# joshspeagle/dynesty

Measured on AMD Instinct MI355X. Metric: proposals/sec + ellipsoid-rebuilds/sec, 25-D corr-Normal nlive=2000 (multi/rwalk), higher is better.
Workload: dtype f64; 1 GPU; C2 x 64 independent runs per GPU (C5 shard); per step and run: 1 MultiEllipsoid rebuild + enlarge 1.25 + 4 queue fills of K=512 walkers x 45 rwalk steps (= one bound-update interval at the queue size that passes the ln Z gate); live sets uniform inside the likelihood contour; ndim=25, nlive=2000, walks=45, queue_size=512, runs_per_gpu=64, tap_point=A (kernel boundary), rebuild_in_step=True, rng=PCG64 + ziggurat, stream-identical to numpy.random.Generator (parity mode)

## Files before the change

### dynesty_amd/csrc/rebuild.hip

```cpp
#include <math.h>
#include <stdlib.h>

#include "ctx.h"
#include <type_traits>
#include <vector>
#include "eig_wave.h"
#include "rebuild_plan.h"

using namespace dh;
using namespace dh_plan;
using dh_eig::jacobi_wave;
using dh_eig::sort_eigs_wave;
using dh_eig::wave_sync;

namespace {

constexpr double kRoundDelta = 1e-3;
constexpr double kMaxCond = 1e12;
constexpr double kEigMult = 10.0;
constexpr int kNTries = 100;

struct Node {
  int start, count;
  int parent, child0, child1;
// ... 248 lines not shown
  const int m = (D + 1) / 2, P = 2 * m;
  lds_double* const ja0 = (lds_double*)L.JA[0];
  lds_double* const ja1 = (lds_double*)L.JA[1];
  lds_double* const jv0 = (lds_double*)L.JV[0];
  lds_double* const jv1 = (lds_double*)L.JV[1];
  bool bad = false;
  double amax = 0.0;
  for (int e = t; e < D * D; e += kThreads) {
    const int i = e / D, j = e - i * D;
    const double v = L.A[i * LD + j];
    if (!isfinite(v)) bad = true;
    amax = fmax(amax, fabs(v));
  }
  if (__syncthreads_or(bad ? 1 : 0)) return false;
  amax = block_reduce_max(amax, L.red);
  const int ex = amax > 0.0 ? ilogb(amax) + 1 : 0;
  for (int e = t; e < P * P; e += kThreads) {
    const int i = e / P, j = e - i * P;
    ja0[i * JLD + j] = (i < D && j < D) ? ldexp(L.A[i * LD + j], -ex) : 0.0;
    jv0[i * JLD + j] = (i == j && i < D) ? 1.0 : 0.0;
  }
  __syncthreads();
  const int nslots = m * m > kThreads ? 2 : 1;
  int ra[2], ca[2], dra[2], drb[2], dca[2], dcb[2], srcl[2];
  bool on[2];
#pragma unroll
  for (int sl = 0; sl < 2; ++sl) {
    const int blk = t + sl * kThreads;
    on[sl] = blk < m * m;
    const int kr = blk / m, kc = blk - kr * m;
    const int wave_base = blk & ~63;
    int l = (on[sl] ? kr : 0) - wave_base % m;
    if (l < 0) l += m;
    srcl[sl] = l;
    ra[sl] = on[sl] ? 2 * kr : 0;
    ca[sl] = 2 * kc;
    dra[sl] = jacobi_dest(ra[sl], m);
    drb[sl] = jacobi_dest(ra[sl] + 1, m);
    dca[sl] = jacobi_dest(2 * kc, m);
    dcb[sl] = jacobi_dest(2 * kc + 1, m);
  }
  int cur = 0;
  int dpos = (D & 1) ? D : -1;
  for (int sweep = 0; sweep < 60; ++sweep) {
    const lds_double* Ac = cur ? ja1 : ja0;
    double off = 0.0, dia = 0.0;
#pragma unroll
    for (int sl = 0; sl < 2; ++sl)
      if (on[sl]) {
        const int r0 = ra[sl], c0 = ca[sl];
        const double x00 = Ac[r0 * JLD + c0], x01 = Ac[r0 * JLD + c0 + 1];
        const double x10 = Ac[(r0 + 1) * JLD + c0], x11 = Ac[(r0 + 1) * JLD + c0 + 1];
        if (r0 == c0) {
          dia = fma(x00, x00, fma(x11, x11, dia));
          off = fma(x01, x01, fma(x10, x10, off));
        } else {
          off = fma(x00, x00, fma(x01, x01, fma(x10, x10, fma(x11, x11, off))));
        }
      }
    off = wave_sum(off);
    dia = wave_sum(dia);
    if ((t & 63) == 0) {
      L.red[t >> 6] = off;
      L.red[8 + (t >> 6)] = dia;
    }
    __syncthreads();
    off = L.red[0] + L.red[1] + L.red[2] + L.red[3];
    dia = L.red[8] + L.red[9] + L.red[10] + L.red[11];
    __syncthreads();
    if (!(off > 1e-31 * dia)) break;
    for (int r = 0; r < P - 1; ++r) {
      const lds_double* As = cur ? ja1 : ja0;
      const lds_double* Vs = cur ? jv1 : jv0;
      lds_double* Ad = cur ? ja0 : ja1;
      lds_double* Vd = cur ? jv0 : jv1;
#pragma unroll
      for (int sl = 0; sl < 2; ++sl) {
        if (sl >= nslots) break;
        const int c0 = ca[sl], c1 = c0 + 1;
        double cc, sc;
        jacobi_rotation(As[c0 * JLD + c0], As[c1 * JLD + c1], As[c0 * JLD + c1], cc, sc);
        const double cr = __shfl(cc, srcl[sl]), sr = __shfl(sc, srcl[sl]);
        if (on[sl]) {
          const int r0 = ra[sl], r1 = r0 + 1;
          const double x00 = As[r0 * JLD + c0], x01 = As[r0 * JLD + c1];
          const double x10 = As[r1 * JLD + c0], x11 = As[r1 * JLD + c1];
          const double v00 = Vs[r0 * JLD + c0], v01 = Vs[r0 * JLD + c1];
          const double v10 = Vs[r1 * JLD + c0], v11 = Vs[r1 * JLD + c1];
          const double y00 = cr * x00 - sr * x10, y01 = cr * x01 - sr * x11;
          const double y10 = sr * x00 + cr * x10, y11 = sr * x01 + cr * x11;
          double z00 = cc * y00 - sc * y01, z01 = sc * y00 + cc * y01;
          double z10 = cc * y10 - sc * y11, z11 = sc * y10 + cc * y11;
          if (r0 == c0) z01 = z10 = 0.0;
          Ad[dra[sl] * JLD + dca[sl]] = z00;
          Ad[dra[sl] * JLD + dcb[sl]] = z01;
          Ad[drb[sl] * JLD + dca[sl]] = z10;
          Ad[drb[sl] * JLD + dcb[sl]] = z11;
          Vd[r0 * JLD + dca[sl]] = cc * v00 - sc * v01;
          Vd[r0 * JLD + dcb[sl]] = sc * v00 + cc * v01;
          Vd[r1 * JLD + dca[sl]] = cc * v10 - sc * v11;
          Vd[r1 * JLD + dcb[sl]] = sc * v10 + cc * v11;
        }
      }
      if (dpos >= 0) dpos = jacobi_dest(dpos, m);
      cur ^= 1;
      __syncthreads();
    }
  }
  const lds_double* Af = cur ? ja1 : ja0;
  const lds_double* Vf = cur ? jv1 : jv0;
  for (int e = t; e < P * P; e += kThreads) {
    const int i = e / P, a = e - i * P;
    if (a == dpos || i >= D) continue;
    const int col = a - ((dpos >= 0 && a > dpos) ? 1 : 0);
    L.V[i * LD + col] = Vf[i * JLD + a];
    if (i == 0) L.A[col * LD + col] = ldexp(Af[a * JLD + a], ex);
  }
  __syncthreads();
  return true;
}

__device__ __forceinline__ double ld_agent(const double* p) {
  return __hip_atomic_load(p, __ATOMIC_RELAXED, __HIP_MEMORY_SCOPE_AGENT);
}
__device__ __forceinline__ void st_agent(double* p, double v) {
  __hip_atomic_store(p, v, __ATOMIC_RELAXED, __HIP_MEMORY_SCOPE_AGENT);
}
__device__ __forceinline__ int ld_agent_i(const int* p) {
  return __hip_atomic_load(p, __ATOMIC_RELAXED, __HIP_MEMORY_SCOPE_AGENT);
}
__device__ __forceinline__ void st_agent_i(int* p, int v) {
  __hip_atomic_store(p, v, __ATOMIC_RELAXED, __HIP_MEMORY_SCOPE_AGENT);
}
__device__ __forceinline__ double sel_ld(const double* base, int off, bool ok) {
  const double v = base[ok ? off : 0];
  return ok ? v : 0.0;
}
__device__ __forceinline__ double ld_c(const Lds& L, const double* p) { return L.coh ? ld_agent(p) : *p; }
__device__ __forceinline__ void st_c(const Lds& L, double* p, double v) {
  if (L.coh)
    st_agent(p, v);
  else
    *p = v;
}
__device__ __forceinline__ int ld_ci(const Lds& L, const int* p) { return L.coh ? ld_agent_i(p) : *p; }
__device__ __forceinline__ void st_ci(const Lds& L, int* p, int v) {
  if (L.coh)
    st_agent_i(p, v);
  else
    *p = v;
}

constexpr int kStageBatch = 8;
template <int NT = kThreads, int SB = kStageBatch, bool IDX_LDS = false>
__device__ __forceinline__ void stage_tile(const Lds& L, const double* __restrict__ pts,
                                           const int* __restrict__ perm, int start, int cnt, int D,
                                           int how) {
  const int j = threadIdx.x & (L.DP - 1);
  const int p0 = threadIdx.x >> L.DPlog, pstep = NT >> L.DPlog;
  if (L.c_pts == pts && L.c_start == start && L.c_cnt == cnt) {
    if (L.c_how == how) return;
    if (L.c_how == 0 && how == 1) {
      if (j < D) {
        const double mj = L.mean[j];
        for (int p = p0; p < cnt; p += pstep) L.tile[p * L.LD + j] -= mj;
      }
      L.c_how = 1;
      __syncthreads();
      return;
    }
  }
  const double mj = (how == 1 && j < D) ? L.mean[j] : 0.0;
  const double sj = (how == 2 && j < D) ? L.scale[j] : 1.0;
  constexpr int SB2 = 10;
  for (int c0 = 0; c0 < cnt; c0 += L.ibuf_cap) {
    const int cc = min(L.ibuf_cap, cnt - c0);
    if (c0) __syncthreads();
    for (int p = threadIdx.x; p < cc; p += NT) L.ibuf[p] = ld_ci(L, perm + start + c0 + p) * D;
    __syncthreads();
    if (j < D) {
      for (int pb = p0; pb < cc; pb += SB2 * pstep) {
        double x[SB2];
#pragma unroll
        for (int k = 0; k < SB2; ++k) {
          const int p = pb + k * pstep;
          x[k] = pts[(unsigned)(L.ibuf[p < cc ? p : 0] + j)];
        }
#pragma unroll
        for (int k = 0; k < SB2; ++k) {
          const int p = pb + k * pstep;
          if (p < cc) {
            double v = x[k];
            if (how == 1) v -= mj;
            if (how == 2) v = v / sj;
            L.tile[(c0 + p) * L.LD + j] = v;
          }
        }
      }
    }
  }
  L.c_pts = pts;
  L.c_start = start;
  L.c_cnt = cnt;
  L.c_how = how;
  __syncthreads();
}

__device__ __forceinline__ void node_mean(const Lds& L, const double* pts, const int* perm, int start, int count, int D) {
  const int t = threadIdx.x;
  const int G = kThreads / D > 0 ? kThreads / D : 1;
  const int j = t % D, g = t / D;
  double total = 0.0;
  for (int base = 0; base < count; base += L.TP) {
    const int cnt = min(L.TP, count - base);
    stage_tile(L, pts, perm, start + base, cnt, D, 0);
    double acc = 0.0;
    if (g < G && t < G * D)
      for (int p = g; p < cnt; p += G) acc += L.tile[p * L.LD + j];
    L.red[t] = acc;
    __syncthreads();
    if (t < D) {
      double s = 0.0;
      for (int gg = 0; gg < G; ++gg) s += L.red[gg * D + t];
      total += s;
    }
    __syncthreads();
  }
  if (t < D) L.mean[t] = total / (double)count;
  __syncthreads();
}

__device__ void node_std(const Lds& L, const double* pts, const int* perm, int start, int count, int D) {
  node_mean(L, pts, perm, start, count, D);
  const int t = threadIdx.x;
  const int G = kThreads / D > 0 ? kThreads / D : 1;
  const int j = t % D, g = t / D;
  double total = 0.0;
  for (int base = 0; base < count; base += L.TP) {
    const int cnt = min(L.TP, count - base);
    stage_tile(L, pts, perm, start + base, cnt, D, 1);
    double acc = 0.0;
    if (g < G && t < G * D)
      for (int p = g; p < cnt; p += G) {
        const double x = L.tile[p * L.LD + j];
        acc = fma(x, x, acc);
      }
    L.red[t] = acc;
    __syncthreads();
    if (t < D) {
      double s = 0.0;
      for (int gg = 0; gg < G; ++gg) s += L.red[gg * D + t];
      total += s;
    }
    __syncthreads();
  }
  if (t < D) L.scale[t] = sqrt(total / (double)count);
  __syncthreads();
}

typedef double mfma_acc __attribute__((ext_vector_type(4)));
constexpr int kMfmaMinDim = 10;
#define DH_MFMA_F64(a, b, c) __builtin_amdgcn_mfma_f64_16x16x4f64((a), (b), (c), 0, 0, 0)
#define DH_MFMA_F64_4X4(a, b, c) __builtin_amdgcn_mfma_f64_4x4x4f64((a), (b), (c), 0, 0, 0)

__device__ __forceinline__ void tile_cov_accumulate(const Lds& L, int cnt, int D, mfma_acc (&acc)[6], int wsel = -1) {
  const int t = threadIdx.x, lane = t & 63, w = wsel >= 0 ? wsel : (t >> 6), LD = L.LD;
  const int nb = (D + 15) >> 4;
  const int lj = lane & 15, lk = lane >> 4;
  const bool v0 = lj < D, v1 = 16 + lj < D, v2 = 32 + lj < D;
  const int pend = min(cnt, w * 64 + 64);
  for (int p0 = w * 64; p0 < pend; p0 += 4) {
    const int p = p0 + lk;
    const bool pv = p < cnt;
    const int ro = p * LD + lj;
    const double f0 = sel_ld(L.tile, ro, pv && v0);
    acc[0] = DH_MFMA_F64(f0, f0, acc[0]);
    if (nb > 1) {
      const double f1 = sel_ld(L.tile, ro + 16, pv && v1);
      acc[1] = DH_MFMA_F64(f0, f1, acc[1]);
      acc[2] = DH_MFMA_F64(f1, f1, acc[2]);
      if (nb > 2) {
        const double f2 = sel_ld(L.tile, ro + 32, pv && v2);
        acc[3] = DH_MFMA_F64(f0, f2, acc[3]);
        acc[4] = DH_MFMA_F64(f1, f2, acc[4]);
        acc[5] = DH_MFMA_F64(f2, f2, acc[5]);
      }
    }
  }
}

__device__ __forceinline__ void cov_fold_waves(const Lds& L, int D, const mfma_acc (&acc)[6]) {
  const int t = threadIdx.x, lane = t & 63, w = t >> 6, LD = L.LD;
  const int nb = (D + 15) >> 4;
  const int lj = lane & 15, lk = lane >> 4;
  for (int wv = 0; wv < kThreads / 64; ++wv) {
    if (w == wv) {
#pragma unroll
      for (int b = 0; b < 6; ++b) {
        const int ib = b == 0 ? 0 : b == 1 ? 0 : b == 2 ? 1 : b == 3 ? 0 : b == 4 ? 1 : 2;
        const int jb = b == 0 ? 0 : b == 1 ? 1 : b == 2 ? 1 : 2;
        if (jb < nb) {
#pragma unroll
          for (int r = 0; r < 4; ++r) {
            const int i = ib * 16 + lk + 4 * r, j = jb * 16 + lj;
            if (i < D && j < D) {
              double v = acc[b][r];
              if (wv > 0) v += L.A[i * LD + j];
              L.A[i * LD + j] = v;
            }
          }
        }
      }
    }
    __syncthreads();
  }
}

template <int NT = kThreads>
__device__ __forceinline__ void cov_finalize(const Lds& L, int D, double inv) {
  for (int e = threadIdx.x; e < D * D; e += NT) {
    const int i = e / D, j = e - i * D;
    if (i <= j) {
      const double c = L.A[i * L.LD + j] * inv;
      L.A[i * L.LD + j] = c;
      L.A[j * L.LD + i] = c;
    }
  }
  __syncthreads();
}

__device__ __forceinline__ bool cov_fold_finalize_all(const Lds& L, int D, const mfma_acc (&acc)[6], double inv,
                                                      double* cov_g) {
  const int t = threadIdx.x, lane = t & 63, w = t >> 6, LD = L.LD;
  const int nb = (D + 15) >> 4;
  const int lj = lane & 15, lk = lane >> 4;
  double* mine = L.A + (size_t)w * D * LD;
#pragma unroll
  for (int b = 0; b < 6; ++b) {
    const int ib = b == 0 ? 0 : b == 1 ? 0 : b == 2 ? 1 : b == 3 ? 0 : b == 4 ? 1 : 2;
    const int jb = b == 0 ? 0 : b == 1 ? 1 : b == 2 ? 1 : 2;
    if (jb < nb) {
#pragma unroll
      for (int r = 0; r < 4; ++r) {
        const int i = ib * 16 + lk + 4 * r, j = jb * 16 + lj;
        if (i <= j && j < D) mine[i * LD + j] = acc[b][r];
      }
    }
  }
  __syncthreads();
  bool bad = false;
  for (int e = t; e < D * D; e += kThreads) {
    const int i = e / D, j = e - i * D;
    if (i <= j) {
      const int o = i * LD + j, ot = j * LD + i;
// ... 751 lines not shown
  if constexpr (FAST) {
    double logdet = 0.0;
    const double* cov_keep = nullptr;
    if (fused != 2 && spd_fast(L, cov_g, D, a.mode == 0 && count >= 4 * D, &logdet, &cov_keep, fused == 1)) {
      const double fmx = node_fmax(L, pts, perm, start, count, D);
      PH_ADD(3);
      if (fmx > 1.0 - kRoundDelta) logdet += (double)D * log(fmx / (1.0 - kRoundDelta));
      *fmax_out = fmin(fmx, 1.0 - kRoundDelta);
      if (cov_keep != nullptr) return ellipsoid_finish_fast(L, a, es, cov_g, cov_keep, fmx, logdet, logvol_out);
      ellipsoid_rescale(L, cov_g, D, fmx);
      return ellipsoid_store_fast(L, a, es, cov_g, logdet, logvol_out);
    }
    if constexpr (CHILD) return kDeferred;
    __syncthreads();
    for (int pass = 0; pass < 2; ++pass) {
      const bool good = regularize<false>(L, cov_g, D);
      const double fmx = node_fmax(L, pts, perm, start, count, D);
      if (pass == 0) ellipsoid_rescale(L, cov_g, D, fmx);
      if (pass == 1 && fmx >= 1.0) return DH_ERR_CONTAIN;
      *fmax_out = pass == 0 ? fmin(fmx, 1.0 - kRoundDelta) : fmx;
      if (good) break;
    }
    const int rc = ellipsoid_store(L, a, es, cov_g, logvol_out);
    return rc == DH_OK ? kFullRecord : rc;
  } else {
    for (int pass = 0; pass < 2; ++pass) {
      const bool good = regularize(L, cov_g, D);
      PH_ADD(2);
      const double fmx = node_fmax(L, pts, perm, start, count, D);
      PH_ADD(3);
      if (pass == 0) ellipsoid_rescale(L, cov_g, D, fmx);
      if (pass == 1 && fmx >= 1.0) return DH_ERR_CONTAIN;
      *fmax_out = pass == 0 ? fmin(fmx, 1.0 - kRoundDelta) : fmx;
      if (good) break;
    }
    return ellipsoid_store(L, a, es, cov_g, logvol_out);
  }
}


constexpr int kBarSleep = 4;
__device__ __forceinline__ void drain_stores() {
  __builtin_amdgcn_s_waitcnt(0x0F70);
}

typedef double dh_d2 __attribute__((ext_vector_type(2)));
__device__ __forceinline__ void st_agent16(double* p, double v, unsigned long long tag) {
  dh_d2 x;
  x.x = v;
  x.y = __longlong_as_double((long long)tag);
  asm volatile("global_store_dwordx4 %0, %1, off sc1\n\ts_nop 1" ::"v"(p), "v"(x) : "memory");
}
__device__ __forceinline__ void ld_agent16x8(const double* const (&p)[8], dh_d2 (&v)[8]) {
  asm volatile(
      "global_load_dwordx4 %0, %8, off sc1\n\t"
      "global_load_dwordx4 %1, %9, off sc1\n\t"
      "global_load_dwordx4 %2, %10, off sc1\n\t"
      "global_load_dwordx4 %3, %11, off sc1\n\t"
      "global_load_dwordx4 %4, %12, off sc1\n\t"
      "global_load_dwordx4 %5, %13, off sc1\n\t"
      "global_load_dwordx4 %6, %14, off sc1\n\t"
      "global_load_dwordx4 %7, %15, off sc1\n\t"
      "s_waitcnt vmcnt(0)"
      : "=&v"(v[0]), "=&v"(v[1]), "=&v"(v[2]), "=&v"(v[3]), "=&v"(v[4]), "=&v"(v[5]), "=&v"(v[6]), "=&v"(v[7])
      : "v"(p[0]), "v"(p[1]), "v"(p[2]), "v"(p[3]), "v"(p[4]), "v"(p[5]), "v"(p[6]), "v"(p[7])
      : "memory");
}

template <bool MAXOP = false>
__device__ __forceinline__ double tagged_partner_reduce(const double* base, size_t stride, int col, int np,
                                                        unsigned long long tag, bool* ok) {
  double acc = MAXOP ? -INFINITY : 0.0;
  for (int pp0 = 0; pp0 < np && *ok; pp0 += 8) {
    const double* ptr[8];
    dh_d2 v[8];
#pragma unroll
    for (int uu = 0; uu < 8; ++uu) ptr[uu] = base + ((size_t)min(pp0 + uu, np - 1) * stride + col) * 2;
    for (int spins = 0;; ++spins) {
      ld_agent16x8(ptr, v);
      bool all = true;
#pragma unroll
      for (int uu = 0; uu < 8; ++uu) all = all && (unsigned long long)__double_as_longlong(v[uu].y) == tag;
      if (all) break;
      if (spins > (1 << 18)) {
        *ok = false;
        break;
      }
      __builtin_amdgcn_s_sleep(1);
    }
#pragma unroll
    for (int uu = 0; uu < 8; ++uu) {
      if (MAXOP)
        acc = pp0 + uu < np ? fmax(acc, v[uu].x) : acc;
      else
        acc += pp0 + uu < np ? v[uu].x : 0.0;
    }
  }
  return acc;
}

__device__ __forceinline__ bool parts_barrier(int* bar, int target) {
  __shared__ int ok_flag;
  drain_stores();
  __syncthreads();
  if (threadIdx.x == 0) {
    __hip_atomic_fetch_add(bar, 1, __ATOMIC_RELAXED, __HIP_MEMORY_SCOPE_AGENT);
    int ok = 1;
    long long spins = 0;
    while (__hip_atomic_load(bar, __ATOMIC_RELAXED, __HIP_MEMORY_SCOPE_AGENT) < target) {
      __builtin_amdgcn_s_sleep(kBarSleep);
      if (++spins > (1ll << 20)) {
        ok = 0;
        break;
      }
    }
    ok_flag = ok;
  }
  __syncthreads();
  return ok_flag != 0;
}

template <bool NB3>
__device__ __forceinline__ void kmeans_label_sums(const Lds& L, unsigned long long sel, double& o0, double& o1, double& o2) {
  const int lane = threadIdx.x & 63, w = threadIdx.x >> 6, LD = L.LD;
  const int lj = lane & 15, lk = lane >> 4;
  double a0 = 0.0, a1 = 0.0, a2 = 0.0, b0 = 0.0, b1 = 0.0, b2 = 0.0;
  const unsigned long long mine = sel >> lk;
  const double* base = L.tile + (w * 64 + lk) * LD + lj;
#pragma unroll 1
  for (int h = 0; h < 2; ++h) {
#pragma unroll
    for (int g = 0; g < 4; ++g) {
      const int g8 = h * 4 + g;
      const double ind = ((mine >> (8 * g8)) & 1ull) ? 1.0 : 0.0;
      const double indb = ((mine >> (8 * g8 + 4)) & 1ull) ? 1.0 : 0.0;
      const double* row = base + g8 * 8 * LD;
      const double* rowb = row + 4 * LD;
      a0 = DH_MFMA_F64_4X4(ind, row[0], a0);
      b0 = DH_MFMA_F64_4X4(indb, rowb[0], b0);
      a1 = DH_MFMA_F64_4X4(ind, row[16], a1);
      b1 = DH_MFMA_F64_4X4(indb, rowb[16], b1);
      if constexpr (NB3) {
        a2 = DH_MFMA_F64_4X4(ind, row[32], a2);
        b2 = DH_MFMA_F64_4X4(indb, rowb[32], b2);
      }
    }
  }
  o0 = a0 + b0;
  o1 = a1 + b1;
  o2 = a2 + b2;
}

template <bool NB3>
__device__ __forceinline__ void kmeans_label_sums_chain(const Lds& L, unsigned long long sel, double& o0, double& o1, double& o2) {
  const int lane = threadIdx.x & 63, w = threadIdx.x >> 6, LD = L.LD;
  const int lj = lane & 15, lk = lane >> 4, cb = (w >> 1) * 4;
  double a0 = 0.0, a1 = 0.0, a2 = 0.0;
  const unsigned long long mine = sel >> (lk + cb);
  const double* base = L.tile + ((w & 1) * 64 + cb + lk) * LD + lj;
#pragma unroll 4
  for (int g8 = 0; g8 < 8; ++g8) {
    const double ind = ((mine >> (8 * g8)) & 1ull) ? 1.0 : 0.0;
    const double* row = base + g8 * 8 * LD;
    a0 = DH_MFMA_F64_4X4(ind, row[0], a0);
    a1 = DH_MFMA_F64_4X4(ind, row[16], a1);
    if constexpr (NB3) a2 = DH_MFMA_F64_4X4(ind, row[32], a2);
  }
  o0 = a0;
  o1 = a1;
  o2 = a2;
}

template <int I>
__device__ __forceinline__ double row_bcast_f64(double v) {
  static_assert(I >= 0 && I < 16, "a lane of the row");
  return __builtin_amdgcn_mov_dpp(v, 0x150 + I, 0xF, 0xF, false);
}
template <int J>
__device__ __forceinline__ double sqdist_step(double d, double x, double c0, double c1, double c2) {
  const double e = x - row_bcast_f64<(J & 15)>(J < 16 ? c0 : J < 32 ? c1 : c2);
  return fma(e, e, d);
}
template <int J0, int ND>
__device__ __forceinline__ double sqdist_blocks(const double* x, double d, const double (&xv)[8], double c0, double c1, double c2) {
  constexpr int N = ND - J0 < 8 ? ND - J0 : 8, NN = ND - J0 - 8 < 8 ? ND - J0 - 8 : 8;
  double xn[8] = {0.0, 0.0, 0.0, 0.0, 0.0, 0.0, 0.0, 0.0};
  if constexpr (NN > 0) {
#pragma unroll
    for (int u = 0; u < NN; ++u) xn[u] = x[J0 + 8 + u];
  }
  if constexpr (N > 0) d = sqdist_step<J0 + 0>(d, xv[0], c0, c1, c2);
  if constexpr (N > 1) d = sqdist_step<J0 + 1>(d, xv[1], c0, c1, c2);
  if constexpr (N > 2) d = sqdist_step<J0 + 2>(d, xv[2], c0, c1, c2);
  if constexpr (N > 3) d = sqdist_step<J0 + 3>(d, xv[3], c0, c1, c2);
  if constexpr (N > 4) d = sqdist_step<J0 + 4>(d, xv[4], c0, c1, c2);
  if constexpr (N > 5) d = sqdist_step<J0 + 5>(d, xv[5], c0, c1, c2);
  if constexpr (N > 6) d = sqdist_step<J0 + 6>(d, xv[6], c0, c1, c2);
  if constexpr (N > 7) d = sqdist_step<J0 + 7>(d, xv[7], c0, c1, c2);
  if constexpr (NN > 0)
    return sqdist_blocks<J0 + 8, ND>(x, d, xn, c0, c1, c2);
  else
    return d;
}
template <int ND>
__device__ __forceinline__ double sqdist_chain(const double* x, double c0, double c1, double c2) {
  static_assert(ND >= 1 && ND <= 48, "three registers of sixteen coordinates");
  double xv[8] = {0.0, 0.0, 0.0, 0.0, 0.0, 0.0, 0.0, 0.0};
#pragma unroll
  for (int u = 0; u < (ND < 8 ? ND : 8); ++u) xv[u] = x[u];
  double d = sqdist_blocks<0, ND>(x, 0.0, xv, c0, c1, c2);
  asm volatile("" : "+v"(d));
  return d;
}
#define DH_WIDE_DIMS(X)                                                                                               \
  X(8) X(9) X(10) X(11) X(12) X(13) X(14) X(15) X(16) X(17) X(18) X(19) X(20) X(21) X(22) X(23) X(24) X(25) X(26) X(27) \
  X(28) X(29) X(30) X(31) X(32) X(33) X(34) X(35) X(36) X(37) X(38) X(39) X(40) X(41) X(42) X(43) X(44) X(45) X(46)   \
  X(47) X(48)

__device__ __forceinline__ double readlane_f64(double v, int l) {
  const long long b = __double_as_longlong(v);
  const unsigned lo = (unsigned)__builtin_amdgcn_readlane((int)(unsigned)b, l);
  const unsigned hi = (unsigned)__builtin_amdgcn_readlane((int)(unsigned)((unsigned long long)b >> 32), l);
  return __longlong_as_double((long long)(((unsigned long long)hi << 32) | lo));
}

__device__ __forceinline__ bool kmeans_wide_form(const Lds& L, int D) { return L.TP == 128 && D >= 8 && D <= 48; }

constexpr int kLloydIters = 10;
static_assert(kLloydIters + 1 <= 0xff, "the iteration tag has 8 bits");

template <bool WIDE>
__device__ int node_kmeans_part(const Lds& L, const double* pts, int* perm, int* perm2, int start, int count,
                                int D, const double* es, int q, int np, double* kp0, double* kp1, int* bar,
                                int min_size, unsigned long long tag0, int lvl = 0) {
  LV_T0();
  const int t = threadIdx.x, lane = t & 63, w = t >> 6, LD = L.LD;
  const int DD = D * D, KP = 2 * D + 2;
  const int s0 = start + q * L.TP, cnt = min(L.TP, count - q * L.TP);
  if (t < D) L.sums[t] = ld_c(L, es + D + 3 * DD + t);
  __syncthreads();
  if (t == 0) {
    L.ri[303] = 0;
    int best = 0;
    double bl = L.sums[0];
    for (int k = 1; k < D; ++k)
      if (L.sums[k] > bl) {
        bl = L.sums[k];
        best = k;
      }
    L.ri[301] = best;
  }
  stage_tile(L, pts, perm, s0, cnt, D, 0);
  const int kbest = L.ri[301];
  if (t < D) {
    const double v = ld_c(L, es + D + 2 * DD + t * D + kbest), ct = ld_c(L, es + t);
    L.cen[t] = (ct - v) / L.scale[t];
    L.cen[D + t] = (ct + v) / L.scale[t];
  }
  __syncthreads();
  const int nb = (D + 15) >> 4;
  const int lj = lane & 15, lk = lane >> 4;
  int lb = 0, lb_prev = -1, n0 = 0, c0_tile = 0, last_it = kLloydIters - 1;
  LV_ADD(lvl, 0);
  LV_SET(lvl, 5, np);
  LV_SET(lvl, 6, count);
  PH_T0();
  {
    const int rup = min(L.TP, (cnt + 63) & ~63);
    const int jz = t & (L.DP - 1), pz0 = cnt + (t >> L.DPlog), pzs = kThreads >> L.DPlog;
    if (jz < D)
      for (int pz = pz0; pz < rup; pz += pzs) L.tile[pz * LD + jz] = 0.0;
    __syncthreads();
  }
  unsigned long long m0 = 0ull, m1 = 0ull;
  constexpr bool wide = WIDE;
  const int half = lane >> 5, pw = (w << 5) | (lane & 31);
  const int wu = __builtin_amdgcn_readfirstlane(w);
  const int cg = cnt - (wu & 1) * 64;
  for (int it = 0; it < kLloydIters; ++it) {
    const bool has = wide ? pw < cnt : t < cnt;
    if (wide) {
      if (w * 32 < cnt) {
        const double* cn = L.cen + half * D + (lane & 15);
        const double c0r = cn[0], c1r = cn[16], c2r = cn[32];
        const double* x = L.tile + (has ? pw : 0) * LD;
        double d = 0.0;
        switch (D) {
#define DH_SQD_CASE(N) \
  case N:              \
    d = sqdist_chain<N>(x, c0r, c1r, c2r); \
    break;
          DH_WIDE_DIMS(DH_SQD_CASE)
#undef DH_SQD_CASE
          default: break;
        }
        const double dp = xor_lane<32>(d);
        lb = (half ? d < dp : dp < d) ? 1 : 0;
      }
    } else if (w * 64 < cnt) {
      const double c0l = L.cen[lane < D ? lane : 0], c1l = L.cen[D + (lane < D ? lane : 0)];
      const double* x = L.tile + (has ? t : 0) * LD;
      double d0 = 0.0, d1 = 0.0;
      for (int j0 = 0; j0 < D; j0 += 8) {
        double xv[8];
#pragma unroll
        for (int u = 0; u < 8; ++u) xv[u] = x[min(j0 + u, D - 1)];
#pragma unroll
        for (int u = 0; u < 8; ++u)
          if (j0 + u < D) {
            const double e0 = xv[u] - readlane_f64(c0l, j0 + u), e1 = xv[u] - readlane_f64(c1l, j0 + u);
            d0 = fma(e0, e0, d0);
            d1 = fma(e1, e1, d1);
          }
      }
      lb = d1 < d0 ? 1 : 0;
    }
    LV_ADD(lvl, 8);
    {
      const unsigned long long mv = __ballot(has && lb != lb_prev);
      m1 = __ballot(has && lb == 1);
      if (wide) {
        const int nv = __popc((unsigned)__ballot(has));
        if (lane == 0) {
          L.ri[260 + w] = __popc((unsigned)mv);
          L.ri[264 + w] = nv - __popc((unsigned)m1);
          L.ri[268 + w] = (int)(unsigned)m1;
        }
      } else {
        m0 = __ballot(has && lb == 0);
        if (lane == 0) {
          L.ri[260 + w] = __popcll(mv);
          L.ri[264 + w] = __popcll(m0);
        }
      }
      lb_prev = lb;
    }
    __syncthreads();
    c0_tile = L.ri[264] + L.ri[265] + L.ri[266] + L.ri[267];
    const int ch_tile = L.ri[260] + L.ri[261] + L.ri[262] + L.ri[263];
    if (wide) {
      const int g2 = (wu & 1) * 2;
      m1 = (unsigned long long)(unsigned)L.ri[268 + g2] | ((unsigned long long)(unsigned)L.ri[269 + g2] << 32);
      m0 = ~m1 & (cg >= 64 ? ~0ull : cg > 0 ? (1ull << cg) - 1ull : 0ull);
    }
    PH_ADD(10);
    LV_ADD(lvl, 9);
    double a0 = 0.0, a1 = 0.0, a2 = 0.0;
    if (wide) {
      if (cg > 0) {
        const int li = lane & 3;
        const unsigned long long sel = li == 0 ? m0 : li == 1 ? m1 : 0ull;
        if (nb > 2)
          kmeans_label_sums_chain<true>(L, sel, a0, a1, a2);
        else
          kmeans_label_sums_chain<false>(L, sel, a0, a1, a2);
      }
    } else if (w * 64 < cnt) {
      const int li = lane & 3;
      const unsigned long long sel = li == 0 ? m0 : li == 1 ? m1 : 0ull;
      if (nb > 2)
        kmeans_label_sums<true>(L, sel, a0, a1, a2);
      else
        kmeans_label_sums<false>(L, sel, a0, a1, a2);
    }
    if (lane < 32) {
      double* o = L.kred + (w * 2 + lk) * 48;
      o[lj] = a0;
      if (nb > 1) o[16 + lj] = a1;
      if (nb > 2) o[32 + lj] = a2;
    }
    LV_ADD(lvl, 10);
    __syncthreads();
    PH_ADD(11);
    LV_ADD(lvl, 11);
    double* kp = (it & 1) ? kp1 : kp0;
    if (t < 2 * D) {
      const int c = t >= D ? 1 : 0, j = t - c * D;
      double sum = 0.0;
      if (wide) {
        double gs = 0.0;
        gs += L.kred[(0 * 2 + c) * 48 + j] + L.kred[(2 * 2 + c) * 48 + j];
        gs += L.kred[(1 * 2 + c) * 48 + j] + L.kred[(3 * 2 + c) * 48 + j];
        sum += gs;
      } else {
        for (int g0 = 0; g0 < kThreads / 64; g0 += L.KG) {
          double gs = 0.0;
          for (int wv = g0; wv < g0 + L.KG; ++wv) gs += L.kred[(wv * 2 + c) * 48 + j];
          sum += gs;
        }
      }
      L.sums[c * D + j] = sum;
      if (np == 1) {
        const int nc = c ? count - c0_tile : c0_tile;
        if (nc > 0) L.cen[c * D + j] = sum / (double)nc;
      }
    }
    n0 = c0_tile;
    LV_ADD(lvl, 12);
    if (np > 1) {
      const unsigned long long tag = tag0 + (unsigned long long)(it + 1);
      if (t < KP) {
        const double mine = t < 2 * D ? L.sums[t] : t == 2 * D ? (double)c0_tile : (double)ch_tile;
        st_agent16(kp + ((size_t)q * KP + t) * 2, mine, tag);
        double sum = 0.0;
        bool ok = true;
        for (int pp0 = 0; pp0 < np && ok; pp0 += 8) {
          const double* ptr[8];
          dh_d2 v[8];
#pragma unroll
          for (int uu = 0; uu < 8; ++uu) ptr[uu] = kp + ((size_t)min(pp0 + uu, np - 1) * KP + t) * 2;
          for (int spins = 0;; ++spins) {
            ld_agent16x8(ptr, v);
            bool all = true;
#pragma unroll
            for (int uu = 0; uu < 8; ++uu) all = all && (unsigned long long)__double_as_longlong(v[uu].y) == tag;
            if (all) break;
            if (spins > (1 << 18)) {
              ok = false;
              break;
            }
            __builtin_amdgcn_s_sleep(1);
          }
#pragma unroll
          for (int uu = 0; uu < 8; ++uu) sum += pp0 + uu < np ? v[uu].x : 0.0;
        }
        if (!ok) L.ri[303] = 1;
        L.sums[t] = sum;
      }
      __syncthreads();
      if (L.ri[303]) return -1;
      n0 = (int)L.sums[2 * D];
    }
    LV_ADD(lvl, 13);
    const int moved = np > 1 ? (int)L.sums[2 * D + 1] : ch_tile;
    if (np > 1) {
      const int n1 = count - n0;
      if (t < D) {
        if (n0 > 0) L.cen[t] = L.sums[t] / (double)n0;
        if (n1 > 0) L.cen[D + t] = L.sums[D + t] / (double)n1;
      }
    }
    __syncthreads();
    PH_ADD(12);
    LV_ADD(lvl, 14);
    if (moved == 0) {
      last_it = it;
      break;
    }
  }
  LV_ADD(lvl, 1);
  LV_SET(lvl, 4, last_it + 1);
  if (min(n0, count - n0) < min_size) return n0;
  if (wide) lb = (L.ri[268 + (t >> 5)] >> (t & 31)) & 1;
  const bool valid = t < cnt;
  const unsigned long long pm0 = __ballot(valid && lb == 0);
  const unsigned long long lt = (1ull << lane) - 1ull;
  if (lane == 0) L.ri[256 + w] = __popcll(pm0);
  __syncthreads();
  int before0 = 0;
  for (int wv = 0; wv < w; ++wv) before0 += L.ri[256 + wv];
  const int rank0 = before0 + __popcll(pm0 & lt);
  int off0 = 0, off1 = n0;
  if (np > 1) {
    const double* kp = (last_it & 1) ? kp1 : kp0;
    for (int pp0 = 0; pp0 < q; pp0 += 8) {
      double part[8];
#pragma unroll
      for (int uu = 0; uu < 8; ++uu)
      {
        const double pv8 = ld_agent(kp + ((size_t)min(pp0 + uu, q - 1) * KP + 2 * D) * 2);
        part[uu] = pp0 + uu < q ? pv8 : 0.0;
      }
#pragma unroll
      for (int uu = 0; uu < 8; ++uu)
        if (pp0 + uu < q) {
          off0 += (int)part[uu];
          off1 += L.TP - (int)part[uu];
        }
    }
  }
  if (valid) {
    const int pos = lb == 0 ? off0 + rank0 : off1 + (t - rank0);
    const int src = ld_ci(L, perm + s0 + t);
    if (np > 1 || L.coh)
      st_agent_i(perm2 + start + pos, src);
    else
      perm2[start + pos] = src;
  }
  if (np > 1) {
    if (!parts_barrier(bar, np)) return -1;
    if (valid) st_ci(L, perm + s0 + t, ld_agent_i(perm2 + s0 + t));
  } else if (L.coh) {
    drain_stores();
    __syncthreads();
    if (valid) st_agent_i(perm + s0 + t, ld_agent_i(perm2 + s0 + t));
  } else {
    __threadfence_block();
    __syncthreads();
    if (valid) perm[s0 + t] = perm2[s0 + t];
  }
  LV_ADD(lvl, 2);
  return n0;
}

__device__ __forceinline__ double logaddexp_d(double x, double y) {
  if (x == y) return x + 0.6931471805599453;
  const double d = x - y;
  if (d > 0) return x + log1p(exp(-d));
  if (d <= 0) return y + log1p(exp(d));
  return x + y;
}


__device__ __forceinline__ void carve(Lds& L, unsigned char* smem, int D, int TP = kThreads) {
  L.LD = D | 1;
  L.TP = TP;
  L.c_pts = nullptr;
  L.c_start = L.c_cnt = L.c_how = -1;
  L.coh = false;
  L.KG = kThreads / 64;
  L.DP = 1;
  L.DPlog = 0;
  while (L.DP < D) {
    L.DP <<= 1;
    ++L.DPlog;
  }
  double* p = (double*)smem;
  L.tile = p;
  p += (size_t)L.TP * L.LD;
  L.A = p;
  p += D * L.LD;
  L.V = p;
  p += D * L.LD;
  L.AM = p;
  p += D * L.LD;
  L.AX = p;
  p += D * L.LD;
  L.mean = p;
  p += D;
  L.scale = p;
  p += D;
  L.lam = p;
  p += D;
  L.cen = p;
  p += 2 * D;
  L.sums = p;
  p += 2 * D + 2;
  L.red = p;
  p += kThreads;
  L.rc = p;
  p += 64;
  L.rs = p;
  p += 64;
  L.kred = L.red;
  L.ibuf = (int*)L.red;
  L.ibuf_cap = 2 * (kThreads + 128);
  L.ri = (int*)p;
  L.perm_sort = L.ri + 320;
  const int P = (D + 1) & ~1;
  L.JLD = P | 1;
  const size_t jdbl = 4 * (size_t)P * L.JLD;
  L.j_alias = rebuild_lds_base_bytes(D, TP) + jdbl * 8 > kLdsSeparate;
  double* jb = L.j_alias ? L.tile : (double*)(smem + rebuild_lds_base_bytes(D, TP));
  L.JA[0] = jb;
  L.JA[1] = jb + (size_t)P * L.JLD;
  L.JV[0] = jb + 2 * (size_t)P * L.JLD;
  L.JV[1] = jb + 3 * (size_t)P * L.JLD;
}

__device__ __forceinline__ void carve_split(Lds& L, unsigned char* smem, int D, int TP) {
  L.LD = D | 1;
  L.TP = TP;
  L.c_pts = nullptr;
  L.c_start = L.c_cnt = L.c_how = -1;
  L.coh = false;
  L.KG = kThreads / 64;
  L.DP = 1;
  L.DPlog = 0;
  while (L.DP < D) {
    L.DP <<= 1;
    ++L.DPlog;
  }
  double* p = (double*)smem;
  L.tile = p;
  p += (size_t)TP * L.LD;
  L.scale = p;
  p += D;
  L.cen = p;
  p += 2 * D;
  L.sums = p;
  p += 2 * D + 2;
  L.red = p;
  L.rc = p + kThreads;
  L.rs = L.rc + 64;
  L.kred = L.red;
  L.ibuf = (int*)L.red;
  L.ibuf_cap = 2 * (kThreads + 128);
  p += kThreads + 128;
  L.ri = (int*)p;
  L.perm_sort = L.ri + 320;
  L.A = L.V = L.AM = L.AX = L.mean = L.lam = nullptr;
  L.JA[0] = L.JA[1] = L.JV[0] = L.JV[1] = nullptr;
  L.JLD = 0;
  L.j_alias = false;
}

// ... 1703 lines not shown
```

Measured before the change: 3.034 billion proposals/s.

## Reorder k-means tile rows so each wave's label mask feeds its MFMA chain directly

For the wide k-means split path, the tile is staged with a permuted row order (chain_row). Each wave's 32 points then line up with its own MFMA label-sum chain, so the 32-bit ballot mask is used directly instead of being rebuilt through LDS from neighbouring waves. The seed-axis argmax becomes a wave-level shuffle reduction and is overlapped with tile staging through a mid callback, which removes a serial thread-0 loop and a barrier. The cost is extra index arithmetic, a more complex final label lookup, and the staging cache being disabled for chain-ordered tiles.

```diff
diff --git a/dynesty_amd/csrc/rebuild.hip b/dynesty_amd/csrc/rebuild.hip
--- a/dynesty_amd/csrc/rebuild.hip
+++ b/dynesty_amd/csrc/rebuild.hip
@@ -424,15 +424,23 @@
 }
 
 constexpr int kStageBatch = 8;
-template <int NT = kThreads, int SB = kStageBatch, bool IDX_LDS = false>
+struct StageNoMid {
+  __device__ __forceinline__ void operator()() const {}
+};
+__device__ __forceinline__ int chain_row(int p) { return (p & 64) | ((p & 4) << 3) | ((p >> 1) & 28) | (p & 3); }
+template <int NT = kThreads, int SB = kStageBatch, bool IDX_LDS = false, class Mid = StageNoMid, bool CHAIN_ROWS = false>
 __device__ __forceinline__ void stage_tile(const Lds& L, const double* __restrict__ pts,
                                            const int* __restrict__ perm, int start, int cnt, int D,
-                                           int how) {
+                                           int how, Mid mid = Mid()) {
   const int j = threadIdx.x & (L.DP - 1);
   const int p0 = threadIdx.x >> L.DPlog, pstep = NT >> L.DPlog;
-  if (L.c_pts == pts && L.c_start == start && L.c_cnt == cnt) {
-    if (L.c_how == how) return;
+  if (!CHAIN_ROWS && L.c_pts == pts && L.c_start == start && L.c_cnt == cnt) {
+    if (L.c_how == how) {
+      mid();
+      return;
+    }
     if (L.c_how == 0 && how == 1) {
+      mid();
       if (j < D) {
         const double mj = L.mean[j];
         for (int p = p0; p < cnt; p += pstep) L.tile[p * L.LD + j] -= mj;
@@ -450,6 +458,7 @@
     if (c0) __syncthreads();
     for (int p = threadIdx.x; p < cc; p += NT) L.ibuf[p] = ld_ci(L, perm + start + c0 + p) * D;
     __syncthreads();
+    if (c0 == 0) mid();
     if (j < D) {
       for (int pb = p0; pb < cc; pb += SB2 * pstep) {
         double x[SB2];
@@ -465,13 +474,14 @@
             double v = x[k];
             if (how == 1) v -= mj;
             if (how == 2) v = v / sj;
-            L.tile[(c0 + p) * L.LD + j] = v;
+            L.tile[(CHAIN_ROWS ? chain_row(c0 + p) : c0 + p) * L.LD + j] = v;
           }
         }
       }
     }
   }
-  L.c_pts = pts;
+  if (cnt <= 0) mid();
+  L.c_pts = CHAIN_ROWS ? nullptr : pts;
   L.c_start = start;
   L.c_cnt = cnt;
   L.c_how = how;
@@ -1529,16 +1539,16 @@
 }
 
 template <bool NB3>
-__device__ __forceinline__ void kmeans_label_sums_chain(const Lds& L, unsigned long long sel, double& o0, double& o1, double& o2) {
+__device__ __forceinline__ void kmeans_label_sums_chain(const Lds& L, unsigned sel, double& o0, double& o1, double& o2) {
   const int lane = threadIdx.x & 63, w = threadIdx.x >> 6, LD = L.LD;
-  const int lj = lane & 15, lk = lane >> 4, cb = (w >> 1) * 4;
+  const int lj = lane & 15, lk = lane >> 4;
   double a0 = 0.0, a1 = 0.0, a2 = 0.0;
-  const unsigned long long mine = sel >> (lk + cb);
-  const double* base = L.tile + ((w & 1) * 64 + cb + lk) * LD + lj;
+  const unsigned mine = sel >> lk;
+  const double* base = L.tile + ((w & 1) * 64 + (w >> 1) * 32 + lk) * LD + lj;
 #pragma unroll 4
   for (int g8 = 0; g8 < 8; ++g8) {
-    const double ind = ((mine >> (8 * g8)) & 1ull) ? 1.0 : 0.0;
-    const double* row = base + g8 * 8 * LD;
+    const double ind = ((mine >> (4 * g8)) & 1u) ? 1.0 : 0.0;
+    const double* row = base + g8 * 4 * LD;
     a0 = DH_MFMA_F64_4X4(ind, row[0], a0);
     a1 = DH_MFMA_F64_4X4(ind, row[16], a1);
     if constexpr (NB3) a2 = DH_MFMA_F64_4X4(ind, row[32], a2);
@@ -1601,6 +1611,27 @@
   return __longlong_as_double((long long)(((unsigned long long)hi << 32) | lo));
 }
 
+__device__ __forceinline__ int wave_argmax_first(double v) {
+  int i = threadIdx.x & 63;
+  if (v != v) v = i == 0 ? INFINITY : -INFINITY;
+#define DH_ARGMAX_STEP(S)                                      \
+  {                                                            \
+    const double ov = xor_lane<S>(v);                          \
+    const int oi = xor_lane_i32<S>(i);                         \
+    const bool take = ov > v || (ov == v && oi < i);           \
+    v = take ? ov : v;                                         \
+    i = take ? oi : i;                                         \
+  }
+  DH_ARGMAX_STEP(32)
+  DH_ARGMAX_STEP(16)
+  DH_ARGMAX_STEP(8)
+  DH_ARGMAX_STEP(4)
+  DH_ARGMAX_STEP(2)
+  DH_ARGMAX_STEP(1)
+#undef DH_ARGMAX_STEP
+  return __builtin_amdgcn_readfirstlane(i);
+}
+
 __device__ __forceinline__ bool kmeans_wide_form(const Lds& L, int D) { return L.TP == 128 && D >= 8 && D <= 48; }
 
 constexpr int kLloydIters = 10;
@@ -1614,25 +1645,43 @@
   const int t = threadIdx.x, lane = t & 63, w = t >> 6, LD = L.LD;
   const int DD = D * D, KP = 2 * D + 2;
   const int s0 = start + q * L.TP, cnt = min(L.TP, count - q * L.TP);
-  if (t < D) L.sums[t] = ld_c(L, es + D + 3 * DD + t);
-  __syncthreads();
-  if (t == 0) {
-    L.ri[303] = 0;
-    int best = 0;
-    double bl = L.sums[0];
-    for (int k = 1; k < D; ++k)
-      if (L.sums[k] > bl) {
-        bl = L.sums[k];
-        best = k;
-      }
-    L.ri[301] = best;
-  }
-  stage_tile(L, pts, perm, s0, cnt, D, 0);
-  const int kbest = L.ri[301];
-  if (t < D) {
-    const double v = ld_c(L, es + D + 2 * DD + t * D + kbest), ct = ld_c(L, es + t);
-    L.cen[t] = (ct - v) / L.scale[t];
-    L.cen[D + t] = (ct + v) / L.scale[t];
+  if constexpr (WIDE) {
+    if (t == 0) L.ri[303] = 0;
+    const double al = lane < D ? ld_c(L, es + D + 3 * DD + lane) : -INFINITY;
+    double sv = 0.0, sc = 0.0;
+    auto seeds = [&]() {
+      const int kbest = wave_argmax_first(al);
+      if (t < D) {
+        sv = ld_c(L, es + D + 2 * DD + t * D + kbest);
+        sc = ld_c(L, es + t);
+      }
+    };
+    stage_tile<kThreads, kStageBatch, false, decltype(seeds), true>(L, pts, perm, s0, cnt, D, 0, seeds);
+    if (t < D) {
+      L.cen[t] = (sc - sv) / L.scale[t];
+      L.cen[D + t] = (sc + sv) / L.scale[t];
+    }
+  } else {
+    if (t < D) L.sums[t] = ld_c(L, es + D + 3 * DD + t);
+    __syncthreads();
+    if (t == 0) {
+      L.ri[303] = 0;
+      int best = 0;
+      double bl = L.sums[0];
+      for (int k = 1; k < D; ++k)
+        if (L.sums[k] > bl) {
+          bl = L.sums[k];
+          best = k;
+        }
+      L.ri[301] = best;
+    }
+    stage_tile(L, pts, perm, s0, cnt, D, 0);
+    const int kbest = L.ri[301];
+    if (t < D) {
+      const double v = ld_c(L, es + D + 2 * DD + t * D + kbest), ct = ld_c(L, es + t);
+      L.cen[t] = (ct - v) / L.scale[t];
+      L.cen[D + t] = (ct + v) / L.scale[t];
+    }
   }
   __syncthreads();
   const int nb = (D + 15) >> 4;
@@ -1646,21 +1695,26 @@
     const int rup = min(L.TP, (cnt + 63) & ~63);
     const int jz = t & (L.DP - 1), pz0 = cnt + (t >> L.DPlog), pzs = kThreads >> L.DPlog;
     if (jz < D)
-      for (int pz = pz0; pz < rup; pz += pzs) L.tile[pz * LD + jz] = 0.0;
-    __syncthreads();
-  }
-  unsigned long long m0 = 0ull, m1 = 0ull;
+      for (int pz = pz0; pz < rup; pz += pzs) L.tile[(WIDE ? chain_row(pz) : pz) * LD + jz] = 0.0;
+    __syncthreads();
+  }
   constexpr bool wide = WIDE;
-  const int half = lane >> 5, pw = (w << 5) | (lane & 31);
-  const int wu = __builtin_amdgcn_readfirstlane(w);
-  const int cg = cnt - (wu & 1) * 64;
-  for (int it = 0; it < kLloydIters; ++it) {
-    const bool has = wide ? pw < cnt : t < cnt;
-    if (wide) {
-      if (w * 32 < cnt) {
-        const double* cn = L.cen + half * D + (lane & 15);
+  if constexpr (WIDE) {
+    const int half = lane >> 5;
+    const int wu = __builtin_amdgcn_readfirstlane(w);
+    const int row0 = (wu & 1) * 64 + (wu >> 1) * 4;
+    const int pw = row0 + ((lane & 28) << 1) + (lane & 3);
+    const bool has = pw < cnt;
+    const bool wave_has = row0 < cnt;
+    const unsigned valid = (unsigned)__ballot(has);
+    constexpr int KS = 48;
+    int* cw = L.ri + 260;
+    double* kr = L.kred;
+    for (int it = 0; it < kLloydIters; ++it) {
+      if (wave_has) {
+        const double* cn = L.cen + half * D + lj;
         const double c0r = cn[0], c1r = cn[16], c2r = cn[32];
-        const double* x = L.tile + (has ? pw : 0) * LD;
+        const double* x = L.tile + (has ? (wu & 1) * 64 + (wu >> 1) * 32 + (lane & 31) : 0) * LD;
         double d = 0.0;
         switch (D) {
 #define DH_SQD_CASE(N) \
@@ -1674,161 +1728,250 @@
         const double dp = xor_lane<32>(d);
         lb = (half ? d < dp : dp < d) ? 1 : 0;
       }
-    } else if (w * 64 < cnt) {
-      const double c0l = L.cen[lane < D ? lane : 0], c1l = L.cen[D + (lane < D ? lane : 0)];
-      const double* x = L.tile + (has ? t : 0) * LD;
-      double d0 = 0.0, d1 = 0.0;
-      for (int j0 = 0; j0 < D; j0 += 8) {
-        double xv[8];
-#pragma unroll
-        for (int u = 0; u < 8; ++u) xv[u] = x[min(j0 + u, D - 1)];
-#pragma unroll
-        for (int u = 0; u < 8; ++u)
-          if (j0 + u < D) {
-            const double e0 = xv[u] - readlane_f64(c0l, j0 + u), e1 = xv[u] - readlane_f64(c1l, j0 + u);
-            d0 = fma(e0, e0, d0);
-            d1 = fma(e1, e1, d1);
+      LV_ADD(lvl, 8);
+      const unsigned mv = (unsigned)__ballot(has && lb != lb_prev);
+      const unsigned m1 = (unsigned)__ballot(has && lb == 1);
+      if (lane == 0) {
+        cw[w] = __popc(mv);
+        cw[4 + w] = __popc(valid) - __popc(m1);
+        cw[8 + w] = (int)m1;
+      }
+      lb_prev = lb;
+      PH_ADD(10);
+      LV_ADD(lvl, 9);
+      double a0 = 0.0, a1 = 0.0, a2 = 0.0;
+      if (wave_has) {
+        const int li = lane & 3;
+        const unsigned sel = li == 0 ? (valid & ~m1) : li == 1 ? m1 : 0u;
+        if (nb > 2)
+          kmeans_label_sums_chain<true>(L, sel, a0, a1, a2);
+        else
+          kmeans_label_sums_chain<false>(L, sel, a0, a1, a2);
+      }
+      if (lane < 32) {
+        double* o = kr + (w * 2 + lk) * KS;
+        o[lj] = a0;
+        if (nb > 1) o[16 + lj] = a1;
+        if (nb > 2) o[32 + lj] = a2;
+      }
+      LV_ADD(lvl, 10);
+      __syncthreads();
+      PH_ADD(11);
+      LV_ADD(lvl, 11);
+      const int c0_tile = cw[4] + cw[5] + cw[6] + cw[7];
+      const int ch_tile = cw[0] + cw[1] + cw[2] + cw[3];
+      int moved;
+      if (np == 1) {
+        n0 = c0_tile;
+        moved = ch_tile;
+        if (t < 2 * D) {
+          const int c = t >= D ? 1 : 0, j = t - c * D;
+          const double* kc = kr + c * KS + j;
+          double gs = 0.0, sum = 0.0;
+          gs += kc[0] + kc[4 * KS];
+          gs += kc[2 * KS] + kc[6 * KS];
+          sum += gs;
+          const int nc = c ? count - c0_tile : c0_tile;
+          if (nc > 0) L.cen[c * D + j] = sum / (double)nc;
+        }
+        LV_ADD(lvl, 12);
+        LV_ADD(lvl, 13);
+      } else {
+        double* kp = (it & 1) ? kp1 : kp0;
+        const unsigned long long tag = tag0 + (unsigned long long)(it + 1);
+        if (t < KP) {
+          double mine;
+          if (t < 2 * D) {
+            const int c = t >= D ? 1 : 0, j = t - c * D;
+            const double* kc = kr + c * KS + j;
+            double gs = 0.0, fs = 0.0;
+            gs += kc[0] + kc[4 * KS];
+            gs += kc[2 * KS] + kc[6 * KS];
+            fs += gs;
+            mine = fs;
+          } else {
+            mine = t == 2 * D ? (double)c0_tile : (double)ch_tile;
           }
-      }
-      lb = d1 < d0 ? 1 : 0;
-    }
-    LV_ADD(lvl, 8);
-    {
-      const unsigned long long mv = __ballot(has && lb != lb_prev);
-      m1 = __ballot(has && lb == 1);
-      if (wide) {
-        const int nv = __popc((unsigned)__ballot(has));
-        if (lane == 0) {
-          L.ri[260 + w] = __popc((unsigned)mv);
-          L.ri[264 + w] = nv - __popc((unsigned)m1);
-          L.ri[268 + w] = (int)(unsigned)m1;
+          LV_ADD(lvl, 12);
+          st_agent16(kp + ((size_t)q * KP + t) * 2, mine, tag);
+          double sum = 0.0;
+          bool ok = true;
+          for (int pp0 = 0; pp0 < np && ok; pp0 += 8) {
+            const double* ptr[8];
+            dh_d2 v[8];
+#pragma unroll
+            for (int uu = 0; uu < 8; ++uu) ptr[uu] = kp + ((size_t)min(pp0 + uu, np - 1) * KP + t) * 2;
+            for (int spins = 0;; ++spins) {
+              ld_agent16x8(ptr, v);
+              bool all = true;
+#pragma unroll
+              for (int uu = 0; uu < 8; ++uu) all = all && (unsigned long long)__double_as_longlong(v[uu].y) == tag;
+              if (all) break;
+              if (spins > (1 << 18)) {
+                ok = false;
+                break;
+              }
+              __builtin_amdgcn_s_sleep(1);
+            }
+#pragma unroll
+            for (int uu = 0; uu < 8; ++uu) sum += pp0 + uu < np ? v[uu].x : 0.0;
+          }
+          if (!ok) L.ri[303] = 1;
+          L.sums[t] = sum;
         }
-      } else {
+        __syncthreads();
+        if (L.ri[303]) return -1;
+        LV_ADD(lvl, 13);
+        n0 = (int)L.sums[2 * D];
+        moved = (int)L.sums[2 * D + 1];
+        if (t < D) {
+          const int n1 = count - n0;
+          if (n0 > 0) L.cen[t] = L.sums[t] / (double)n0;
+          if (n1 > 0) L.cen[D + t] = L.sums[D + t] / (double)n1;
+        }
+      }
+      __syncthreads();
+      PH_ADD(12);
+      LV_ADD(lvl, 14);
+      if (moved == 0) {
+        last_it = it;
+        break;
+      }
+    }
+  } else {
+    unsigned long long m0 = 0ull, m1 = 0ull;
+    for (int it = 0; it < kLloydIters; ++it) {
+      const bool has = t < cnt;
+      if (w * 64 < cnt) {
+        const double c0l = L.cen[lane < D ? lane : 0], c1l = L.cen[D + (lane < D ? lane : 0)];
+        const double* x = L.tile + (has ? t : 0) * LD;
+        double d0 = 0.0, d1 = 0.0;
+        for (int j0 = 0; j0 < D; j0 += 8) {
+          double xv[8];
+#pragma unroll
+          for (int u = 0; u < 8; ++u) xv[u] = x[min(j0 + u, D - 1)];
+#pragma unroll
+          for (int u = 0; u < 8; ++u)
+            if (j0 + u < D) {
+              const double e0 = xv[u] - readlane_f64(c0l, j0 + u), e1 = xv[u] - readlane_f64(c1l, j0 + u);
+              d0 = fma(e0, e0, d0);
+              d1 = fma(e1, e1, d1);
+            }
+        }
+        lb = d1 < d0 ? 1 : 0;
+      }
+      LV_ADD(lvl, 8);
+      {
+        const unsigned long long mv = __ballot(has && lb != lb_prev);
+        m1 = __ballot(has && lb == 1);
         m0 = __ballot(has && lb == 0);
         if (lane == 0) {
           L.ri[260 + w] = __popcll(mv);
           L.ri[264 + w] = __popcll(m0);
         }
-      }
-      lb_prev = lb;
-    }
-    __syncthreads();
-    c0_tile = L.ri[264] + L.ri[265] + L.ri[266] + L.ri[267];
-    const int ch_tile = L.ri[260] + L.ri[261] + L.ri[262] + L.ri[263];
-    if (wide) {
-      const int g2 = (wu & 1) * 2;
-      m1 = (unsigned long long)(unsigned)L.ri[268 + g2] | ((unsigned long long)(unsigned)L.ri[269 + g2] << 32);
-      m0 = ~m1 & (cg >= 64 ? ~0ull : cg > 0 ? (1ull << cg) - 1ull : 0ull);
-    }
-    PH_ADD(10);
-    LV_ADD(lvl, 9);
-    double a0 = 0.0, a1 = 0.0, a2 = 0.0;
-    if (wide) {
-      if (cg > 0) {
+        lb_prev = lb;
+      }
+      __syncthreads();
+      c0_tile = L.ri[264] + L.ri[265] + L.ri[266] + L.ri[267];
+      const int ch_tile = L.ri[260] + L.ri[261] + L.ri[262] + L.ri[263];
+      PH_ADD(10);
+      LV_ADD(lvl, 9);
+      double a0 = 0.0, a1 = 0.0, a2 = 0.0;
+      if (w * 64 < cnt) {
         const int li = lane & 3;
         const unsigned long long sel = li == 0 ? m0 : li == 1 ? m1 : 0ull;
         if (nb > 2)
-          kmeans_label_sums_chain<true>(L, sel, a0, a1, a2);
+          kmeans_label_sums<true>(L, sel, a0, a1, a2);
         else
-          kmeans_label_sums_chain<false>(L, sel, a0, a1, a2);
-      }
-    } else if (w * 64 < cnt) {
-      const int li = lane & 3;
-      const unsigned long long sel = li == 0 ? m0 : li == 1 ? m1 : 0ull;
-      if (nb > 2)
-        kmeans_label_sums<true>(L, sel, a0, a1, a2);
-      else
-        kmeans_label_sums<false>(L, sel, a0, a1, a2);
-    }
-    if (lane < 32) {
-      double* o = L.kred + (w * 2 + lk) * 48;
-      o[lj] = a0;
-      if (nb > 1) o[16 + lj] = a1;
-      if (nb > 2) o[32 + lj] = a2;
-    }
-    LV_ADD(lvl, 10);
-    __syncthreads();
-    PH_ADD(11);
-    LV_ADD(lvl, 11);
-    double* kp = (it & 1) ? kp1 : kp0;
-    if (t < 2 * D) {
-      const int c = t >= D ? 1 : 0, j = t - c * D;
-      double sum = 0.0;
-      if (wide) {
-        double gs = 0.0;
-        gs += L.kred[(0 * 2 + c) * 48 + j] + L.kred[(2 * 2 + c) * 48 + j];
-        gs += L.kred[(1 * 2 + c) * 48 + j] + L.kred[(3 * 2 + c) * 48 + j];
-        sum += gs;
-      } else {
+          kmeans_label_sums<false>(L, sel, a0, a1, a2);
+      }
+      if (lane < 32) {
+        double* o = L.kred + (w * 2 + lk) * 48;
+        o[lj] = a0;
+        if (nb > 1) o[16 + lj] = a1;
+        if (nb > 2) o[32 + lj] = a2;
+      }
+      LV_ADD(lvl, 10);
+      __syncthreads();
+      PH_ADD(11);
+      LV_ADD(lvl, 11);
+      double* kp = (it & 1) ? kp1 : kp0;
+      if (t < 2 * D) {
+        const int c = t >= D ? 1 : 0, j = t - c * D;
+        double sum = 0.0;
         for (int g0 = 0; g0 < kThreads / 64; g0 += L.KG) {
           double gs = 0.0;
           for (int wv = g0; wv < g0 + L.KG; ++wv) gs += L.kred[(wv * 2 + c) * 48 + j];
           sum += gs;
         }
-      }
-      L.sums[c * D + j] = sum;
-      if (np == 1) {
-        const int nc = c ? count - c0_tile : c0_tile;
-        if (nc > 0) L.cen[c * D + j] = sum / (double)nc;
-      }
-    }
-    n0 = c0_tile;
-    LV_ADD(lvl, 12);
-    if (np > 1) {
-      const unsigned long long tag = tag0 + (unsigned long long)(it + 1);
-      if (t < KP) {
-        const double mine = t < 2 * D ? L.sums[t] : t == 2 * D ? (double)c0_tile : (double)ch_tile;
-        st_agent16(kp + ((size_t)q * KP + t) * 2, mine, tag);
-        double sum = 0.0;
-        bool ok = true;
-        for (int pp0 = 0; pp0 < np && ok; pp0 += 8) {
-          const double* ptr[8];
-          dh_d2 v[8];
-#pragma unroll
-          for (int uu = 0; uu < 8; ++uu) ptr[uu] = kp + ((size_t)min(pp0 + uu, np - 1) * KP + t) * 2;
-          for (int spins = 0;; ++spins) {
-            ld_agent16x8(ptr, v);
-            bool all = true;
-#pragma unroll
-            for (int uu = 0; uu < 8; ++uu) all = all && (unsigned long long)__double_as_longlong(v[uu].y) == tag;
-            if (all) break;
-            if (spins > (1 << 18)) {
-              ok = false;
-              break;
+        L.sums[c * D + j] = sum;
+        if (np == 1) {
+          const int nc = c ? count - c0_tile : c0_tile;
+          if (nc > 0) L.cen[c * D + j] = sum / (double)nc;
+        }
+      }
+      n0 = c0_tile;
+      LV_ADD(lvl, 12);
+      if (np > 1) {
+        const unsigned long long tag = tag0 + (unsigned long long)(it + 1);
+        if (t < KP) {
+          const double mine = t < 2 * D ? L.sums[t] : t == 2 * D ? (double)c0_tile : (double)ch_tile;
+          st_agent16(kp + ((size_t)q * KP + t) * 2, mine, tag);
+          double sum = 0.0;
+          bool ok = true;
+          for (int pp0 = 0; pp0 < np && ok; pp0 += 8) {
+            const double* ptr[8];
+            dh_d2 v[8];
+#pragma unroll
+            for (int uu = 0; uu < 8; ++uu) ptr[uu] = kp + ((size_t)min(pp0 + uu, np - 1) * KP + t) * 2;
+            for (int spins = 0;; ++spins) {
+              ld_agent16x8(ptr, v);
+              bool all = true;
+#pragma unroll
+              for (int uu = 0; uu < 8; ++uu) all = all && (unsigned long long)__double_as_longlong(v[uu].y) == tag;
+              if (all) break;
+              if (spins > (1 << 18)) {
+                ok = false;
+                break;
+              }
+              __builtin_amdgcn_s_sleep(1);
             }
-            __builtin_amdgcn_s_sleep(1);
+#pragma unroll
+            for (int uu = 0; uu < 8; ++uu) sum += pp0 + uu < np ? v[uu].x : 0.0;
           }
-#pragma unroll
-          for (int uu = 0; uu < 8; ++uu) sum += pp0 + uu < np ? v[uu].x : 0.0;
+          if (!ok) L.ri[303] = 1;
+          L.sums[t] = sum;
         }
-        if (!ok) L.ri[303] = 1;
-        L.sums[t] = sum;
+        __syncthreads();
+        if (L.ri[303]) return -1;
+        n0 = (int)L.sums[2 * D];
+      }
+      LV_ADD(lvl, 13);
+      const int moved = np > 1 ? (int)L.sums[2 * D + 1] : ch_tile;
+      if (np > 1) {
+        const int n1 = count - n0;
+        if (t < D) {
+          if (n0 > 0) L.cen[t] = L.sums[t] / (double)n0;
+          if (n1 > 0) L.cen[D + t] = L.sums[D + t] / (double)n1;
+        }
       }
       __syncthreads();
-      if (L.ri[303]) return -1;
-      n0 = (int)L.sums[2 * D];
-    }
-    LV_ADD(lvl, 13);
-    const int moved = np > 1 ? (int)L.sums[2 * D + 1] : ch_tile;
-    if (np > 1) {
-      const int n1 = count - n0;
-      if (t < D) {
-        if (n0 > 0) L.cen[t] = L.sums[t] / (double)n0;
-        if (n1 > 0) L.cen[D + t] = L.sums[D + t] / (double)n1;
-      }
-    }
-    __syncthreads();
-    PH_ADD(12);
-    LV_ADD(lvl, 14);
-    if (moved == 0) {
-      last_it = it;
-      break;
+      PH_ADD(12);
+      LV_ADD(lvl, 14);
+      if (moved == 0) {
+        last_it = it;
+        break;
+      }
     }
   }
   LV_ADD(lvl, 1);
   LV_SET(lvl, 4, last_it + 1);
   if (min(n0, count - n0) < min_size) return n0;
-  if (wide) lb = (L.ri[268 + (t >> 5)] >> (t & 31)) & 1;
+  if (wide) {
+    int tp = t;
+    asm volatile("" : "+v"(tp));
+    lb = (L.ri[268 + ((tp >> 6) & 1) + ((tp >> 1) & 2)] >> (((tp >> 1) & 28) | (tp & 3))) & 1;
+  }
   const bool valid = t < cnt;
   const unsigned long long pm0 = __ballot(valid && lb == 0);
   const unsigned long long lt = (1ull << lane) - 1ull;
```

Result: no change. 3.059 billion proposals/s, median of 6 (+0.8%).
